# OzAmram/CaloDiffusion

Hardware: AMD Instinct MI355X
Metric: sampled showers/sec (Dataset-2, 400-step DDIM) (higher is better)
Workload: dtype f32 (convs: fp32 operands as 2-term fp16 splits on the fp16 MFMA pipe, fp32 accumulate; attention/norms fp32)

## Files before the change

calodiffusion_amd/csrc/conv_internal.h:

```cpp
#pragma once
#include "kernels_conv.h"
#include "split16.h"
#include <cstdio>
#include <cstdlib>
#include <map>
#include <string>

namespace cd {

#define MFMA32(a, b, c) __builtin_amdgcn_mfma_f32_32x32x2f32((a), (b), (c), 0, 0, 0)
#define MFMA_BF16(a, b, c) __builtin_amdgcn_mfma_f32_32x32x16_bf16(__builtin_bit_cast(bf16x8, (a)), __builtin_bit_cast(bf16x8, (b)), (c), 0, 0, 0)

typedef __bf16 bf16x8 __attribute__((ext_vector_type(8)));
typedef __bf16 bf16x2 __attribute__((ext_vector_type(2)));

__device__ __forceinline__ unsigned pack_bf16(float lo, float hi) {
  const bf16x2 v = {(__bf16)lo, (__bf16)hi};
  return __builtin_bit_cast(unsigned, v);
}
__device__ __forceinline__ void split3(const f32x4 x, u32x2& t1, u32x2& t2, u32x2& t3) {
  f32x4 r = x;
  t1 = u32x2{pack_bf16(r[0], r[1]), pack_bf16(r[2], r[3])};
  r[0] -= __uint_as_float(t1[0] << 16); r[1] -= __uint_as_float(t1[0] & 0xffff0000u);
  r[2] -= __uint_as_float(t1[1] << 16); r[3] -= __uint_as_float(t1[1] & 0xffff0000u);
// ... 21 lines not shown
struct ConvTiled3Args {
  ConvKArgs k;
  float* ch_part;
  int* status;
};
void launch_conv_tiled_f32(int VT, int CT, const ConvKArgs& a, dim3 grid, int threads, size_t lds, hipStream_t s);
void launch_conv_tiled_split16(int VT, int CT, int NTERM, const ConvTiled3Args& a, dim3 grid, int threads, size_t lds, hipStream_t s);

struct ConvFlatArgs {
  const float* in0;
  const float* in1;
  int c0, c1;
  const float* wpk;
  const float* bias;
  float* out;
  int D, H, W;
  int Do, Ho, Wo;
  int R;
  int P;
  int cout, CTtot;
  int dbg;
  const float* coef;
  int act;
  float* ch_part;
  int* status = nullptr;
  GnDefer defer;
  int coef_lds_off = 0;
  const unsigned* in_absmax = nullptr;
  const float* add_src = nullptr;
};
bool try_launch_conv3_flat(const float* in0, int c0, const float* in1, int c1, const void* wpk, const float* bias, float* out,
                           int batch, int cout, const ConvGeom& g, hipStream_t s, const ConvFusion& fu,
                           int prec );
bool launch_conv_flat_split16(int VT, int CT, int NTERM, int geo, const ConvFlatArgs& a, dim3 grid, int threads, size_t lds, hipStream_t s);

std::map<std::string, int>& tune_cache();
template <typename F>
int autotune(const std::string& key, int ncand, F&& run, hipStream_t s) {
  auto it = tune_cache().find(key);
  if (it != tune_cache().end()) return it->second;
  hipStreamCaptureStatus st = hipStreamCaptureStatusNone;
  if (getenv("CD_NO_AUTOTUNE") || hipStreamIsCapturing(s, &st) != hipSuccess || st != hipStreamCaptureStatusNone || prof::enabled())
    return -1;
  hipEvent_t e0, e1;
  CD_HIP(hipEventCreate(&e0));
  CD_HIP(hipEventCreate(&e1));
  int best = 0;
  float best_ms = 1e30f;
  for (int i = 0; i < ncand; ++i) {
    run(i);
    CD_HIP(hipEventRecord(e0, s));
    run(i);
    run(i);
    CD_HIP(hipEventRecord(e1, s));
    CD_HIP(hipEventSynchronize(e1));
    float ms = 0.f;
    CD_HIP(hipEventElapsedTime(&ms, e0, e1));
    if (getenv("CD_TUNE_VERBOSE") && atoi(getenv("CD_TUNE_VERBOSE")) > 1) std::fprintf(stderr, "[calodiff autotune]   %s cand %d: %.1f us\n", key.c_str(), i, ms * 500.f);
    if (ms < best_ms) { best_ms = ms; best = i; }
  }
  hipEventDestroy(e0);
  hipEventDestroy(e1);
  tune_cache()[key] = best;
  if (getenv("CD_TUNE_VERBOSE")) std::fprintf(stderr, "[calodiff autotune] %s -> candidate %d (%.1f us)\n", key.c_str(), best, best_ms * 500.f);
  return best;
}

// ... 2 lines not shown
```

calodiffusion_amd/csrc/kernels_conv.hip:

```cpp
#include "conv_internal.h"
#include <cstring>
#include <algorithm>
#include <vector>

namespace cd {

static int g_conv_precision = -1;
static thread_local int tl_conv_precision_override = -1;
void set_conv_precision_override(int p) { tl_conv_precision_override = p; }
int conv_precision() {
  if (tl_conv_precision_override >= 0) return tl_conv_precision_override;
  if (g_conv_precision < 0) {
    const char* e = getenv("CD_CONV_PRECISION");
    g_conv_precision = !e ? PREC_F16X2 : (!strcmp(e, "f32") ? PREC_F32 : (!strcmp(e, "bf16x3") ? PREC_BF16X3 : PREC_F16X2));
  }
  return g_conv_precision;
}
void set_conv_precision(int p) { g_conv_precision = p; }

__device__ __forceinline__ void pack_weights_elem(size_t idx, const float* __restrict__ w, float* __restrict__ wpk, int cout, int cin,
                                                  int taps, int transposed, int flip) {
  const int e = idx & 3, lane = (idx >> 2) & 63, q = (idx >> 8) & 3;
  size_t rest = idx >> 10;
  const int CT = (cout + 31) / 32;
// ... 142 lines not shown
        double per_round = (double)((resident * NW + 3) / 4) * VT;
        const double cost = rounds * per_round + 0.02 * (double)IZ * IH * g.in.w / 32.0 * rounds;
        all.push_back({cost, ConvTile{TZ, TH, NW, VT, lds}});
      }
    }
  }
  CD_REQUIRE(!all.empty(), "no convolution tiling fits in LDS (grid too wide in r?)");
  std::stable_sort(all.begin(), all.end(), [](const auto& x, const auto& y) { return x.first < y.first; });
  std::vector<ConvTile> out;
  for (auto& c : all) {
    out.push_back(c.second);
    if ((int)out.size() >= keep) break;
  }
  return out;
}

ConvKArgs conv_k_args(const ConvGeom& g, const ConvTile& t, const ConvFusion& fu, const float* in0, int c0, const float* in1, int c1,
                      const float* wpk, const float* bias, float* out, int cout) {
  ConvKArgs a;
  a.in0 = in0; a.in1 = in1; a.c0 = c0; a.c1 = c1; a.wpk = wpk; a.bias = bias; a.out = out;
  a.Din = g.in.d; a.Hin = g.in.h; a.Win = g.in.w; a.Do = g.out.d; a.Ho = g.out.h; a.Wo = g.out.w;
  a.KD = g.kd; a.KH = g.kh; a.KW = g.kw; a.SZ = g.sz; a.SH = g.sh; a.SW = g.sw;
  a.TZ = t.TZ; a.TH = t.TH; a.nTZ = (g.out.d + t.TZ - 1) / t.TZ; a.nTH = (g.out.h + t.TH - 1) / t.TH;
  a.IZ = (t.TZ - 1) * g.sz + g.kd; a.IH = (t.TH - 1) * g.sh + g.kh;
  a.cout = cout; a.CTtot = cout / 32; a.coef = fu.coef; a.act = fu.act;
  return a;
}
}

void launch_conv_mfma(const float* in0, int c0, const float* in1, int c1, const float* wpk, const float* bias, float* out,
                      int batch, int cout, const ConvGeom& g, hipStream_t s, const ConvFusion& fu_in) {
  CD_REQUIRE((!fu_in.coef && !fu_in.defer.part) || c1 == 0, "conv: a fused input normalisation needs a single (non-concatenated) source");
  if (fu_in.units) *fu_in.units = 0;
  CD_REQUIRE(c0 % 32 == 0 && c1 % 32 == 0 && c0 > 0, "conv: channel counts must be multiples of 32");
  CD_REQUIRE(cout % 32 == 0, "conv: output channels must be a multiple of 32");
  CD_REQUIRE(g.kw <= 4, "conv: r kernel extent > 4 unsupported");
  const int CTtot = cout / 32;
  const int CT = CTtot <= 3 ? CTtot : 2;
  CD_REQUIRE(CTtot % CT == 0, "conv: unsupported output channel count");
  char cat[128];
  std::snprintf(cat, sizeof cat, "conv%dx%dx%d_s%d C%d->%d @%dx%dx%d", g.kd, g.kh, g.kw, g.sh, c0 + c1, cout, g.in.d, g.in.h, g.in.w);
  const double taps = (double)g.kd * g.kh * g.kw;
  prof::Scope scope(cat, s, 2.0 * taps * (c0 + c1) * cout * (double)g.out.vox() * batch,
                    4.0 * batch * ((double)g.in.vox() * (c0 + c1) + (double)g.out.vox() * cout));
  ConvFusion fu = fu_in;
  auto materialise = [&]() {
    if (!fu.defer.part) return;
    if (fu.defer.coef_out) fu.coef_buf = fu.defer.coef_out;
    CD_REQUIRE(fu.coef_buf, "conv: deferred normalisation needs a coefficient buffer for kernels without the prologue");
    launch_gn_finalize(fu.defer.part, fu.defer.units, fu.defer.gamma, fu.defer.beta, fu.defer.add, fu.defer.add_ld, fu.coef_buf, batch,
                       fu.defer.C, fu.defer.groups, fu.defer.vox, s, fu.defer.stat_out);
    fu.coef = fu.coef_buf;
    fu.defer = GnDefer();
  };
  auto tiled = [&](int nterm, const void* w) -> bool {
    std::vector<ConvTile> cand;
    for (const ConvTile& t : conv_tile_candidates(g, batch, CT, 14, nterm == 2 ? 80 : (nterm == 3 ? 96 : 144)))
      if (nterm == 0 || (nterm == 2 ? t.VT * CT <= 2 : (t.VT <= 4 && !(CT == 3 && t.VT > 2)))) cand.push_back(t);
    if (cand.empty()) return false;
    auto launch = [&](const ConvTile& t) {
      ConvTiled3Args a3;
      a3.k = conv_k_args(g, t, fu, in0, c0, in1, c1, (const float*)w, bias, out, cout);
      const int units = a3.k.nTZ * a3.k.nTH;
      dim3 grid((unsigned)(batch * units), (unsigned)(CTtot / CT));
      if (nterm == 0) {
        launch_conv_tiled_f32(t.VT, CT, a3.k, grid, t.NW * 64, t.lds, s);
        return;
      }
      a3.status = fu.status;
      const int64_t cap = (g.out.vox() + 31) / 32;
      a3.ch_part = (fu.ch_part && units <= cap) ? fu.ch_part : nullptr;
      if (fu.units) *fu.units = a3.ch_part ? units : 0;
      const size_t red = (size_t)t.NW * CT * 32 * 2 * 4;
      launch_conv_tiled_split16(t.VT, CT, nterm, a3, grid, t.NW * 64, std::max(t.lds, red), s);
    };
    char key[192];
    if (nterm) std::snprintf(key, sizeof key, "tiled_%s %s b%d", nterm == 2 ? "f16x2" : "bf16x3", cat, batch);
    else std::snprintf(key, sizeof key, "tiled %s b%d", cat, batch);
    const int pick = autotune(key, (int)cand.size(), [&](int i) { launch(cand[i]); }, s);
    launch(cand[pick < 0 ? 0 : pick]);
    return true;
  };

  const int prec = conv_precision();
  const void* w_bf16x3 = prec != PREC_F32 ? fu.wpk_bf16x3 : nullptr;
  const void* w_f16x2 = w_bf16x3 && prec == PREC_F16X2 ? (const char*)w_bf16x3 + packed_bf16x3_bytes(c0 + c1, cout, g.kd * g.kh * g.kw) : nullptr;
  if (w_f16x2 && try_launch_conv_zslide(in0, c0, in1, c1, w_f16x2, bias, out, batch, cout, g, s, fu)) return;
  if (w_f16x2 && try_launch_conv_small(in0, c0, in1, c1, w_f16x2, bias, out, batch, cout, g, s, fu)) return;
  if (w_f16x2 && try_launch_conv3_flat(in0, c0, in1, c1, w_f16x2, bias, out, batch, cout, g, s, fu, 2)) return;
  materialise();
  if (w_bf16x3 && try_launch_conv3_flat(in0, c0, in1, c1, w_bf16x3, bias, out, batch, cout, g, s, fu, 3)) return;
  if (try_launch_conv3_flat(in0, c0, in1, c1, wpk, bias, out, batch, cout, g, s, fu, 0)) return;
  if (w_f16x2 && !fu.in_absmax && tiled(2, w_f16x2)) return;
  if (w_bf16x3 && tiled(3, w_bf16x3)) return;
  tiled(0, wpk);
}

}
```

calodiffusion_amd/csrc/kernels_conv_flat.hip:

```cpp
#include "conv_internal.h"
#include "gn_defer.h"
#include <vector>

namespace cd {

template <int VT, int CT>
__global__ void __launch_bounds__(512, (VT * CT <= 2 ? 3 : 2)) conv3_flat_kernel(ConvFlatArgs a) {
  extern __shared__ __attribute__((aligned(16))) float lds[];
  const int tid = threadIdx.x, lane = tid & 63, wave = tid >> 6, nthreads = blockDim.x;
  const int b = blockIdx.y;
  const int ct0 = blockIdx.z * CT;
  const int HW = a.H * a.W;
  const int vox = a.D * HW;
  const int v0 = blockIdx.x * a.R;
  const int vend = min(v0 + a.R, vox);
  const int zA = v0 / HW - 1;
  const int zB = (vend - 1) / HW + 1;
  const int nstage = (zB - zA + 1) * HW;
  const int NZ = a.P * HW;
  const int half = lane >> 5, col = lane & 31;
  if (tid < 16) lds[NZ * 16 + tid] = 0.f;

  int nb[VT], rowm[VT], rowp[VT], ooff[VT];
  unsigned wmask[VT];
  bool any_valid = false;
#pragma unroll
  for (int vt = 0; vt < VT; ++vt) {
    const int v = v0 + (wave * VT + vt) * 32 + col;
    const bool valid = v < vend;
    const int vv = valid ? v : v0;
    const int r = vv % HW;
    const int h = r / a.W, w = r - h * a.W;
    nb[vt] = vv - zA * HW;
    rowm[vt] = (h == 0 ? a.H - 1 : -1) * a.W;
// ... 447 lines not shown
  }
  CD_FLAT_CASE(1, 1) CD_FLAT_CASE(2, 1) CD_FLAT_CASE(3, 1) CD_FLAT_CASE(4, 1)
  CD_FLAT_CASE(1, 2) CD_FLAT_CASE(2, 2) CD_FLAT_CASE(3, 2) CD_FLAT_CASE(4, 2)
  CD_FLAT_CASE(1, 3) CD_FLAT_CASE(2, 3)
#undef CD_FLAT_CASE
  return false;
}
}

bool try_launch_conv3_flat(const float* in0, int c0, const float* in1, int c1, const void* wpk, const float* bias, float* out,
                           int batch, int cout, const ConvGeom& g, hipStream_t s, const ConvFusion& fu, int prec) {
  const bool bf16x3 = prec != 0;
  if (getenv("CD_NO_FLAT")) return false;
  int geo = -1;
  if (g.kd == 3 && g.kh == 3 && g.kw == 3 && g.sz == 1 && g.sh == 1 && g.sw == 1) geo = 0;
  else if (g.kd == 3 && g.kh == 4 && g.kw == 4 && g.sh == 2 && g.sw == 2 && (g.sz == 1 || g.sz == 2)) geo = g.sz == 2 ? 1 : 2;
  else if (g.kd == 4 && g.kh == 4 && g.kw == 4 && g.sh == 2 && g.sw == 2 && g.sz == 2) geo = 3;
  if (geo < 0 || (geo != 0 && !bf16x3)) return false;
  const Dims3 d = g.in;
  const int CTtot = cout / 32;
  const int CTmax = CTtot <= 3 ? CTtot : 2;
  if (CTtot % CTmax) return false;
  const int HW = d.h * d.w, HWo = g.out.h * g.out.w;
  const size_t vox_bytes = prec == 3 ? 96 : (prec == 2 ? 80 : 64);
  auto planes = [&](int NT) { return ((32 * NT - 1) / HWo + 1) * g.sz + g.kd; };
  auto args_for = [&](int NT) {
    ConvFlatArgs a;
    a.in0 = in0; a.in1 = in1; a.c0 = c0; a.c1 = c1; a.wpk = (const float*)wpk; a.bias = bias; a.out = out;
    a.D = d.d; a.H = d.h; a.W = d.w; a.Do = g.out.d; a.Ho = g.out.h; a.Wo = g.out.w;
    a.R = 32 * NT; a.P = planes(NT); a.cout = cout; a.CTtot = CTtot;
    a.coef = fu.coef; a.act = fu.act; a.ch_part = fu.ch_part;
    return a;
  };
  auto launch = [&](int NT, int VT, int CT) -> bool {
    if (VT < 0) {
      const int NLW = -VT;
      ConvFlatArgs a = args_for(NT);
      a.dbg = 0;
      const size_t lds = 2 * ((size_t)a.P * HW + 1) * 96 + (size_t)NT * CT * 64 * 4;
      const int ups = (int)((g.out.vox() + a.R - 1) / a.R);
      const int total = ups * batch;
      const int nblk = total < 256 ? total : 256;
      dim3 grid((unsigned)nblk, 1, (unsigned)(CTtot / CT));
      if (fu.units) *fu.units = ups;
      const int threads = (NT + NLW) * 64;
      switch (CT) {
        case 1: launch_ws_inst<1>(a, grid, threads, lds, NLW, ups, total, s, geo); break;
        case 2: launch_ws_inst<2>(a, grid, threads, lds, NLW, ups, total, s, geo); break;
        case 3: launch_ws_inst<3>(a, grid, threads, lds, NLW, ups, total, s, geo); break;
        default: return false;
      }
      return true;
    }
    ConvFlatArgs a = args_for(NT);
    a.dbg = getenv("CD_FLAT_DBG") ? atoi(getenv("CD_FLAT_DBG")) : 0;
    a.status = fu.status; a.in_absmax = fu.in_absmax;
    a.add_src = prec >= 2 && !bias ? fu.add_src : nullptr;
    size_t lds = ((size_t)a.P * HW + 1) * vox_bytes;
    const size_t red = (size_t)(NT / VT) * CT * 32 * 2 * 4;
    if (lds < red) lds = red;
    if (fu.defer.part) {
      lds = (lds + 15) & ~(size_t)15;
      a.defer = fu.defer;
      a.coef_lds_off = (int)lds;
      lds += (size_t)fu.defer.C * 16 + gn_defer_scratch_bytes(fu.defer.C);
      if (lds > 160 * 1024) return false;
    }
    dim3 grid((unsigned)((g.out.vox() + a.R - 1) / a.R), (unsigned)batch, (unsigned)(CTtot / CT));
    if (fu.units) *fu.units = (int)grid.x;
    const int threads = (NT / VT) * 64;
    const bool launched = prec != 0 ? launch_conv_flat_split16(VT, CT, prec, geo, a, grid, threads, lds, s)
                                    : launch_conv_flat_f32(VT, CT, a, grid, threads, lds, s);
    if (!launched) return false;
    if (a.add_src && fu.add_done) *fu.add_done = 1;
    return true;
  };
  if (const char* ov = getenv("CD_FLAT_TILE")) {
    int nt, vt;
    if (sscanf(ov, "%d,%d", &nt, &vt) == 2 && nt % vt == 0 && nt / vt <= 8 && vt * CTmax <= 8 &&
        ((size_t)planes(nt) * HW + 1) * vox_bytes <= 160 * 1024 && (prec != 2 || vt * CTmax <= 4))
      return launch(nt, vt, CTmax);
  }
  static const int kCand[][2] = {{8, 2}, {4, 1}, {8, 1}, {12, 3}, {16, 2}, {16, 4}, {4, 2}, {6, 2}, {6, 3}, {2, 1},
                                 {3, 1}, {1, 1}, {2, 2}, {12, 2}, {8, 4}, {6, 1}, {3, 3}};
  struct Cand { int nt, vt, ct; };
  std::vector<Cand> cand;
  const bool small = g.out.vox() * batch <= 64 * 1024;
  for (int pass = 0; pass < (small && CTmax > 1 ? 2 : 1); ++pass) {
    const int CT = pass == 0 ? CTmax : 1;
    for (auto& c : kCand) {
      const int NT = c[0], VT = c[1];
      if (VT * CT > 8 || (CT == 3 && VT > 2)) continue;
      if (prec == 2 && VT * CT > 4) continue;
      static const bool no_extra_waves = getenv("CD_FLAT_NO_EXTRA_WAVES") != nullptr;
      const bool extra_ok = !no_extra_waves && g.out.vox() <= 128 && VT == 1 && NT <= 8;
      if ((int64_t)32 * (NT - 1) >= g.out.vox() && !extra_ok) continue;
      if (((size_t)planes(NT) * HW + 1) * vox_bytes > 150 * 1024) continue;
      if (pass == 1 && NT > 4) continue;
      cand.push_back({NT, VT, CT});
    }
  }
  if (prec == 3 && !getenv("CD_NO_WS")) {
    static const int kWs[][2] = {{8, 4}, {8, 2}, {4, 2}, {4, 4}, {8, 3}, {6, 2}, {2, 2}, {3, 1}, {1, 1}, {2, 1}};
    for (auto& c : kWs) {
      const int NMW = c[0], NLW = c[1];
      if ((int64_t)32 * (NMW - 1) >= g.out.vox()) continue;
      const size_t lds = 2 * ((size_t)planes(NMW) * HW + 1) * 96 + (size_t)NMW * CTmax * 64 * 4;
      if (lds > 160 * 1024 - 256) continue;
      cand.push_back({NMW, -NLW, CTmax});
    }
  }
  if (cand.empty()) return false;
  char key[192];
  std::snprintf(key, sizeof key, "flat%s g%d %dx%dx%d c%d+%d->%d b%d", prec == 3 ? "_bf16x3" : (prec == 2 ? "_f16x2" : "_f32"), geo,
                d.d, d.h, d.w, c0, c1, cout, batch);
  const int pick = autotune(key, (int)cand.size(), [&](int i) { launch(cand[i].nt, cand[i].vt, cand[i].ct); }, s);
  const Cand& c = cand[pick < 0 ? 0 : pick];
  return launch(c.nt, c.vt, c.ct);
}

}
```

calodiffusion_amd/csrc/kernels_conv_flat16.hip:

```cpp
#include "conv_internal.h"
#include "gn_defer.h"

namespace cd {

template <int VT, int CT, int KD, int KH, int KW, int SZ, int SXY, int NTERM>
__global__ void __launch_bounds__(512, (VT * CT * (NTERM == 2 ? 2 : 1) <= 2 ? 3 : 2)) conv3_flat_bf16x3_kernel(ConvFlatArgs a) {
  extern __shared__ __attribute__((aligned(16))) float lds[];
  char* ldsb = (char*)lds;
  constexpr int T = KD * KH * KW;
  constexpr int VB = NTERM == 3 ? 96 : 80;
  constexpr int WS = 64 * NTERM;
  const int tid = threadIdx.x, lane = tid & 63, wave = tid >> 6, nthreads = blockDim.x;
  const int b = blockIdx.y;
  const int ct0 = blockIdx.z * CT;
  const int HW = a.H * a.W;
  const int vox = a.D * HW;
  const int HWo = a.Ho * a.Wo;
  const int voxo = a.Do * HWo;
  const int v0 = blockIdx.x * a.R;
  const int vend = min(v0 + a.R, voxo);
  const float inv_hwo = 1.f / (float)HWo, inv_wo = 1.f / (float)a.Wo;
  auto fdiv = [](int x, float inv) { return (int)(((float)x + 0.5f) * inv); };
  const int zA = fdiv(v0, inv_hwo) * SZ - 1;
  const int zB = fdiv(vend - 1, inv_hwo) * SZ + KD - 2;
  const int nstage = (zB - zA + 1) * HW;
  const int NZ = a.P * HW;
  const int half = lane >> 5, col = lane & 31;
  if (a.defer.part) gn_defer_to_lds(a.defer, b, (float*)(ldsb + a.coef_lds_off), ldsb + a.coef_lds_off + a.defer.C * 16);
  const bool normed = a.coef || a.defer.part;
  if (tid < VB / 4) ((float*)(ldsb + (size_t)NZ * VB))[tid] = 0.f;

  int nb[VT], rowoff[VT][KH], ooff[VT];
  unsigned wmask[VT];
  bool any_valid = false;
#pragma unroll
  for (int vt = 0; vt < VT; ++vt) {
    const int v = v0 + (wave * VT + vt) * 32 + col;
    const bool valid = v < vend;
    const int vv = valid ? v : v0;
    const int oz = fdiv(vv, inv_hwo);
    const int r = vv - oz * HWo;
    const int oh = fdiv(r, inv_wo), ow = r - oh * a.Wo;
    const int ih0 = oh * SXY, iw0 = ow * SXY;
    nb[vt] = (oz * SZ - 1 - zA) * HW + ih0 * a.W + iw0;
    unsigned m = 0;
#pragma unroll
    for (int kh = 0; kh < KH; ++kh) {
      int ih = ih0 + kh - 1;
      ih = ih < 0 ? ih + a.H : (ih >= a.H ? ih - a.H : ih);
      ih = ih >= a.H ? ih - a.H : ih;
      rowoff[vt][kh] = (ih - ih0) * a.W;
    }
#pragma unroll
    for (int kw = 0; kw < KW; ++kw) {
      const int iw = iw0 + kw - 1;
      if (valid && iw >= 0 && iw < a.W) m |= 1u << kw;
    }
    wmask[vt] = m;
    ooff[vt] = valid ? v * a.cout : -1;
    any_valid |= valid;
  }
  const bool wave_active = __any(any_valid);

  f32x16 acc[VT][CT], accB[NTERM == 2 ? VT : 1][NTERM == 2 ? CT : 1];
#pragma unroll
  for (int vt = 0; vt < VT; ++vt)
#pragma unroll
    for (int ct = 0; ct < CT; ++ct)
#pragma unroll
      for (int r = 0; r < 16; ++r) {
// ... 6 lines not shown
  if (NTERM == 2 && a.in_absmax) pow2_scale_for(*a.in_absmax, &gscale, &ginv);
  const int nsub = (a.c0 + a.c1) >> 4;
  const int gbase = zA * HW;
  const int nslots = nstage * 4;

  auto tap_voxel = [&](int vt, int tap) -> int {
#ifdef CD_FLAT_ABL_TAPS
    return nb[vt] + tap;
#endif
    const int kz = tap / (KH * KW), kh = (tap / KW) % KH, kw = tap % KW;
    const int n = nb[vt] + kz * HW + rowoff[vt][kh] + kw - 1;
    return ((wmask[vt] >> kw) & 1u) ? n : NZ;
  };

  for (int sc = 0; sc < nsub; ++sc) {
    const float* src;
    int ldc, coff;
    if (sc * 16 < a.c0) {
      src = a.in0; ldc = a.c0; coff = sc * 16;
    } else {
      src = a.in1; ldc = a.c1; coff = sc * 16 - a.c0;
    }
    const int pq = tid & 3;
    src += (size_t)b * vox * ldc + coff + pq * 4;
    f32x4 cf[4];
    if (a.defer.part) {
#pragma unroll
      for (int e = 0; e < 4; ++e) cf[e] = *(const f32x4*)(ldsb + a.coef_lds_off + (sc * 16 + pq * 4 + e) * 16);
    } else if (a.coef) {
#pragma unroll
      for (int e = 0; e < 4; ++e) cf[e] = *(const f32x4*)(a.coef + ((size_t)b * (a.c0 + a.c1) + sc * 16 + pq * 4 + e) * 4);
    }
    __syncthreads();
    for (int s0 = tid; s0 < ((a.dbg & 1) ? 0 : nslots); s0 += 4 * nthreads) {
      f32x4 val[4];
#pragma unroll
      for (int k = 0; k < 4; ++k) {
        const int sidx = s0 + k * nthreads;
        const int g = gbase + (sidx >> 2);
        val[k] = f32x4{0.f, 0.f, 0.f, 0.f};
        if (sidx < nslots && g >= 0 && g < vox) {
          val[k] = *(const f32x4*)(src + (size_t)g * ldc);
          if (normed) {
#pragma unroll
            for (int e = 0; e < 4; ++e) {
              float t = cf[e][0] * val[k][e] + cf[e][1];
              if (a.act) t = cd_fast_silu(t);
              val[k][e] = t + cf[e][2];
            }
          }
        }
      }
#pragma unroll
      for (int k = 0; k < 4; ++k) {
        const int sidx = s0 + k * nthreads;
        if (sidx < nslots) {
          char* d = ldsb + (size_t)(sidx >> 2) * VB + pq * 8;
          if (NTERM == 3) {
            u32x2 t1, t2, t3;
            split3(val[k], t1, t2, t3);
            *(u32x2*)d = t1;
            *(u32x2*)(d + 32) = t2;
            *(u32x2*)(d + 64) = t3;
          } else {
            const f32x4 vs = val[k] * gscale;
            amax = fmaxf(amax, fmaxf(fmaxf(fabsf(vs[0]), fabsf(vs[1])), fmaxf(fabsf(vs[2]), fabsf(vs[3]))));
            u32x2 t1, t2;
            split2(vs, t1, t2);
            *(u32x2*)d = t1;
            *(u32x2*)(d + 32) = t2;
          }
        }
      }
    }
    __syncthreads();
    if (!wave_active || (a.dbg & 2)) continue;

#pragma unroll
    for (int vt = 0; vt < VT; ++vt) asm volatile("" : "+v"(nb[vt]));

    const u32x4* wq = (const u32x4*)a.wpk + ((size_t)sc * T * a.CTtot + ct0) * WS + lane;
#ifndef CD_FLAT_WD
#define CD_FLAT_WD 3
#endif
#ifndef CD_FLAT_AD
#define CD_FLAT_AD 2
#endif
    constexpr bool DEEP = NTERM == 2;
    constexpr int WD = DEEP ? CD_FLAT_WD : 1, AD = DEEP ? CD_FLAT_AD : 1;
    u32x4 bw[WD + 1][CT][NTERM], av[AD + 1][VT][NTERM];
    auto load_w = [&](int tap) {
#pragma unroll
      for (int ct = 0; ct < CT; ++ct)
#pragma unroll
        for (int t = 0; t < NTERM; ++t) bw[tap % (WD + 1)][ct][t] = wq[((size_t)tap * a.CTtot + ct) * WS + t * 64];
    };
    auto load_a = [&](int tap) {
#pragma unroll
      for (int vt = 0; vt < VT; ++vt) {
        const char* p = ldsb + (size_t)tap_voxel(vt, tap) * VB + half * 16;
#pragma unroll
        for (int t = 0; t < NTERM; ++t) av[tap % (AD + 1)][vt][t] = *(const u32x4*)(p + t * 32);
      }
    };
#pragma unroll
    for (int t0 = 0; t0 < WD; ++t0) load_w(t0);
#pragma unroll
    for (int t0 = 0; t0 < AD; ++t0) load_a(t0);
#pragma unroll
    for (int tap = 0; tap < T; ++tap) {
      if (tap + WD < T) load_w(tap + WD);
      if (tap + AD < T) load_a(tap + AD);
      __builtin_amdgcn_sched_barrier(0);
      const int wc = tap % (WD + 1), ac = tap % (AD + 1);
#pragma unroll
      for (int vt = 0; vt < VT; ++vt)
#pragma unroll
        for (int ct = 0; ct < CT; ++ct) {
          if (NTERM == 3) {
            f32x16 c = acc[vt][ct];
            c = MFMA_BF16(av[ac][vt][NTERM - 1], bw[wc][ct][0], c);
            c = MFMA_BF16(av[ac][vt][1], bw[wc][ct][1], c);
            c = MFMA_BF16(av[ac][vt][0], bw[wc][ct][NTERM - 1], c);
            c = MFMA_BF16(av[ac][vt][1], bw[wc][ct][0], c);
            c = MFMA_BF16(av[ac][vt][0], bw[wc][ct][1], c);
            c = MFMA_BF16(av[ac][vt][0], bw[wc][ct][0], c);
            acc[vt][ct] = c;
          } else {
            acc[vt][ct] = MFMA_F16(av[ac][vt][0], bw[wc][ct][0], acc[vt][ct]);
            accB[vt][ct] = MFMA_F16(av[ac][vt][0], bw[wc][ct][1], accB[vt][ct]);
            accB[vt][ct] = MFMA_F16(av[ac][vt][1], bw[wc][ct][0], accB[vt][ct]);
          }
        }
    }
  }

  if (NTERM == 2) {
#pragma unroll
    for (int vt = 0; vt < VT; ++vt)
#pragma unroll
      for (int ct = 0; ct < CT; ++ct)
#pragma unroll
        for (int r = 0; r < 16; ++r) acc[vt][ct][r] = (acc[vt][ct][r] + accB[vt][ct][r] * (1.f / 2048.f)) * ginv;
  }
  if (NTERM == 2 && a.status && amax > 65504.f) atomicOr(a.status, 1);
  float* outb = a.out + (size_t)b * voxo * a.cout;
  float bv[CT];
#pragma unroll
  for (int ct = 0; ct < CT; ++ct) bv[ct] = a.bias ? a.bias[(ct0 + ct) * 32 + col] : 0.f;
  if (a.add_src) {
    const float* addb = a.add_src + (size_t)b * voxo * a.cout;
#pragma unroll
    for (int vt = 0; vt < VT; ++vt) {
      float ad[16][CT];
#pragma unroll
      for (int r = 0; r < 16; ++r) {
        const int off = __shfl(ooff[vt], (r & 3) + 8 * (r >> 2) + 4 * half, 64);
#pragma unroll
        for (int ct = 0; ct < CT; ++ct) ad[r][ct] = off >= 0 ? addb[off + (ct0 + ct) * 32 + col] : 0.f;
      }
#pragma unroll
      for (int r = 0; r < 16; ++r)
#pragma unroll
        for (int ct = 0; ct < CT; ++ct) acc[vt][ct][r] += ad[r][ct];
    }
  }
#pragma unroll
  for (int vt = 0; vt < VT; ++vt) {
#pragma unroll
    for (int r = 0; r < 16; ++r) {
      const int row = (r & 3) + 8 * (r >> 2) + 4 * half;
      const int off = __shfl(ooff[vt], row, 64);
      if (off >= 0) {
#pragma unroll
        for (int ct = 0; ct < CT; ++ct) outb[off + (ct0 + ct) * 32 + col] = acc[vt][ct][r] + bv[ct];
      }
    }
  }
// ... 9 lines not shown
        const bool ok = __shfl(ooff[vt], row, 64) >= 0;
#pragma unroll
        for (int ct = 0; ct < CT; ++ct) {
          const float v = ok ? acc[vt][ct][r] + bv[ct] : 0.f;
          s1[ct] += v;
          s2[ct] += v * v;
        }
      }
    __syncthreads();
    const int nw = nthreads >> 6;
#pragma unroll
    for (int ct = 0; ct < CT; ++ct) {
      const float t1 = s1[ct] + __shfl_xor(s1[ct], 32, 64), t2 = s2[ct] + __shfl_xor(s2[ct], 32, 64);
      if (half == 0) {
        lds[((wave * CT + ct) * 32 + col) * 2] = t1;
        lds[((wave * CT + ct) * 32 + col) * 2 + 1] = t2;
      }
    }
    __syncthreads();
    for (int i = tid; i < CT * 32; i += nthreads) {
      float t1 = 0.f, t2 = 0.f;
      for (int w = 0; w < nw; ++w) {
        t1 += lds[((w * CT * 32) + i) * 2];
        t2 += lds[((w * CT * 32) + i) * 2 + 1];
      }
      float* dst = a.ch_part + (((size_t)b * gridDim.x + blockIdx.x) * a.cout + ct0 * 32 + i) * 2;
      dst[0] = t1;
      dst[1] = t2;
    }
  }
}

namespace {
template <int VT, int CT, int KD, int KH, int KW, int SZ, int SXY, int NTERM>
void launch_flat3_geo(const ConvFlatArgs& a, dim3 grid, int threads, size_t lds, hipStream_t s) {
  static bool attr_set = false;
  if (!attr_set) {
    CD_HIP(hipFuncSetAttribute((const void*)conv3_flat_bf16x3_kernel<VT, CT, KD, KH, KW, SZ, SXY, NTERM>,
                               hipFuncAttributeMaxDynamicSharedMemorySize, 160 * 1024));
    attr_set = true;
  }
  hipLaunchKernelGGL((conv3_flat_bf16x3_kernel<VT, CT, KD, KH, KW, SZ, SXY, NTERM>), grid, dim3(threads), lds, s, a);
  CD_HIP(hipGetLastError());
}
template <int VT, int CT, int NTERM>
void launch_flat3_inst(const ConvFlatArgs& a, dim3 grid, int threads, size_t lds, hipStream_t s, int geo = 0) {
  if (geo == 0) launch_flat3_geo<VT, CT, 3, 3, 3, 1, 1, NTERM>(a, grid, threads, lds, s);
  else if (geo == 1) launch_flat3_geo<VT, CT, 3, 4, 4, 2, 2, NTERM>(a, grid, threads, lds, s);
  else if (geo == 2) launch_flat3_geo<VT, CT, 3, 4, 4, 1, 2, NTERM>(a, grid, threads, lds, s);
  else launch_flat3_geo<VT, CT, 4, 4, 4, 2, 2, NTERM>(a, grid, threads, lds, s);
}
}

bool launch_conv_flat_split16(int VT, int CT, int NTERM, int geo, const ConvFlatArgs& a, dim3 grid, int threads, size_t lds, hipStream_t s) {
#define CD_FLAT_CASE(V, C)                                                                 \
  if (VT == V && CT == C) {                                                                \
    if (NTERM == 3) launch_flat3_inst<V, C, 3>(a, grid, threads, lds, s, geo);             \
    else if constexpr (V * C <= 4) launch_flat3_inst<V, C, 2>(a, grid, threads, lds, s, geo); \
    else return false;                                                                     \
    return true;                                                                           \
  }
  CD_FLAT_CASE(1, 1) CD_FLAT_CASE(2, 1) CD_FLAT_CASE(3, 1) CD_FLAT_CASE(4, 1)
  CD_FLAT_CASE(1, 2) CD_FLAT_CASE(2, 2) CD_FLAT_CASE(3, 2) CD_FLAT_CASE(4, 2)
  CD_FLAT_CASE(1, 3) CD_FLAT_CASE(2, 3)
#undef CD_FLAT_CASE
  return false;
}

}
```

calodiffusion_amd/csrc/ops.hip:

```cpp
#include "plan_internal.h"

namespace cd {

__global__ void to_cl_kernel(const float* __restrict__ src, float* __restrict__ dst, int channels, int64_t vox) {
  const int b = blockIdx.y;
  const int64_t total = vox * channels;
  for (int64_t i = (int64_t)blockIdx.x * 256 + threadIdx.x; i < total; i += (int64_t)gridDim.x * 256) {
    const int c = (int)(i % channels);
    const int64_t v = i / channels;
    dst[(size_t)b * total + i] = src[(size_t)b * total + (size_t)c * vox + v];
  }
}
__global__ void to_planar_kernel(const float* __restrict__ src, float* __restrict__ dst, int channels, int64_t vox) {
  const int b = blockIdx.y;
  const int64_t total = vox * channels;
  for (int64_t i = (int64_t)blockIdx.x * 256 + threadIdx.x; i < total; i += (int64_t)gridDim.x * 256) {
    const int64_t v = i % vox;
    const int c = (int)(i / vox);
    dst[(size_t)b * total + i] = src[(size_t)b * total + (size_t)v * channels + c];
  }
}
static void launch_transpose_to_cl(const float* ncdhw, float* ndhwc, int batch, int channels, int64_t vox, hipStream_t s) {
  int64_t bx = (vox * channels + 255) / 256;
  if (bx > 1024) bx = 1024;
// ... 6 lines not shown
  hipLaunchKernelGGL(to_planar_kernel, dim3((unsigned)bx, batch), dim3(256), 0, s, ndhwc, ncdhw, channels, vox);
  CD_HIP(hipGetLastError());
}

}

extern "C" {

static AbsmaxWords op_absmax_words(Arena& ws, hipStream_t s) {
  constexpr size_t kWords = 8;
  unsigned* w = ws.get<unsigned>(kWords);
  CD_HIP(hipMemsetAsync(w, 0, sizeof(unsigned) * kWords, s));
  return AbsmaxWords{w, w + kWords};
}
size_t cd_op_scratch_bytes(int batch, int max_channels, int64_t max_voxels) {
  return (size_t)256 * 256 * 64 * 4 * 4 + (size_t)batch * 64 * 64 * 16 + (size_t)batch * max_channels * max_voxels * 4 + (1 << 20);
}

int cd_op_to_channels_last(const float* ncdhw, float* ndhwc, int batch, int channels, int64_t voxels, void* stream) {
  return guarded([&] { launch_transpose_to_cl(ncdhw, ndhwc, batch, channels, voxels, (hipStream_t)stream); });
}
int cd_op_to_ncdhw(const float* ndhwc, float* ncdhw, int batch, int channels, int64_t voxels, void* stream) {
  return guarded([&] { launch_transpose_to_planar(ndhwc, ncdhw, batch, channels, voxels, (hipStream_t)stream); });
}

int cd_op_cyl_conv(const float* x0, int c0, const float* x1, int c1, const float* w, const float* bias, float* y,
                   int batch, int cout, const int32_t dims_in[3], const int32_t kernel[3], const int32_t stride[3],
                   void* scratch, void* stream) {
  return guarded([&] {
    CD_REQUIRE(x0 && w && y && scratch, "null argument");
    hipStream_t s = (hipStream_t)stream;
    const int taps = kernel[0] * kernel[1] * kernel[2];
    float* wpk = (float*)scratch;
    launch_pack_weights(w, wpk, cout, c0 + c1, taps, false, s);
    const Dims3 din{dims_in[0], dims_in[1], dims_in[2]};
    if (taps == 1) {
      PointwiseArgs a;
      a.in0 = x0; a.ld0 = c0; a.c0 = c0; a.in1 = x1; a.ld1 = c1; a.c1 = c1; a.wpk = wpk; a.bias = bias; a.out = y;
      a.batch = batch; a.cout = cout; a.vox = din.vox();
      launch_pointwise(a, s);
    } else {
      CD_REQUIRE(cout % 32 == 0, "cout must be a multiple of 32");
      ConvGeom g;
      g.in = din;
      g.kd = kernel[0]; g.kh = kernel[1]; g.kw = kernel[2]; g.sz = stride[0]; g.sh = stride[1]; g.sw = stride[2];
      g.out = Dims3{(din.d + 2 - g.kd) / g.sz + 1, (din.h + 2 - g.kh) / g.sh + 1, (din.w + 2 - g.kw) / g.sw + 1};
      ConvFusion fu;
      if (taps == 27 || taps == 48) {
        float* w3 = wpk + packed_weight_floats(c0 + c1, cout, taps);
        launch_pack_weights_split16(w, w3, cout, c0 + c1, taps, s);
        fu.wpk_bf16x3 = w3;
      }
      launch_conv_mfma(x0, c0, x1, c1, wpk, bias, y, batch, cout, g, s, fu);
    }
  });
}

int cd_op_zslide_conv(const float* x, int cin, const float* w, const float* bias, float* y, float* ch_part, int* units, int batch,
                      int cout, const int32_t dims[3], int chunks, void* scratch, void* stream) {
  return guarded([&] {
    CD_REQUIRE(x && w && y && ch_part && units && scratch && chunks >= 0, "bad argument");
    CD_REQUIRE(cin % 32 == 0 && cout % 32 == 0, "channel counts must be multiples of 32");
    hipStream_t s = (hipStream_t)stream;
    launch_pack_weights_f16x2(w, scratch, cout, cin, 27, s);
    const Dims3 d{dims[0], dims[1], dims[2]};
    ConvGeom g{d, d, 3, 3, 3, 1, 1, 1};
    ConvFusion fu;
    int u = 0;
    fu.act = 1; fu.ch_part = ch_part; fu.units = &u; fu.zs_chunks = chunks;
    CD_REQUIRE(try_launch_conv_zslide(x, cin, nullptr, 0, scratch, bias, y, batch, cout, g, s, fu) && u > 0,
               "this grid is not eligible for the z-slide kernel");
    *units = u;
  });
}

int cd_op_cyl_conv_transpose(const float* x, const float* w, const float* bias, float* y, int batch, int channels,
                             const int32_t dims_in[3], int kernel_z, int stride_z, const int32_t out_pad[3],
                             void* scratch, void* stream) {
  return guarded([&] {
    CD_REQUIRE(x && w && y && scratch, "null argument");
    CD_REQUIRE(out_pad[0] == 0, "z output padding is always 0 (models.py:339)");
    hipStream_t s = (hipStream_t)stream;
// ... 153 lines not shown
```

Measured before the change: 92.57.

## Add tap-split (split-K over taps) variants of flat f16x2 conv kernel

Adds a KS template parameter to the flat split16 conv kernel so several wave groups each handle a disjoint slice of the kernel taps for the same output tile. Their partial accumulators are reduced through LDS before the epilogue. The variants are offered as extra autotune candidates for the 3x4x4 geometries, to raise parallelism on small-voxel layers. The change also relaxes the channel requirement to multiples of 16 for 4x4 kernels on the f16x2 path. The cost is more LDS use, an extra reduction and barrier step, and a longer autotune search.

```diff
diff --git a/calodiffusion_amd/csrc/conv_internal.h b/calodiffusion_amd/csrc/conv_internal.h
--- a/calodiffusion_amd/csrc/conv_internal.h
+++ b/calodiffusion_amd/csrc/conv_internal.h
@@ -77,7 +77,9 @@
 bool try_launch_conv3_flat(const float* in0, int c0, const float* in1, int c1, const void* wpk, const float* bias, float* out,
                            int batch, int cout, const ConvGeom& g, hipStream_t s, const ConvFusion& fu,
                            int prec );
-bool launch_conv_flat_split16(int VT, int CT, int NTERM, int geo, const ConvFlatArgs& a, dim3 grid, int threads, size_t lds, hipStream_t s);
+bool launch_conv_flat_split16(int VT, int CT, int NTERM, int geo, const ConvFlatArgs& a, dim3 grid, int threads, size_t lds, hipStream_t s,
+                              int KS = 1);
+bool conv_flat_tapsplit_offered(int VT, int CT, int NTERM, int geo, int KS);
 
 std::map<std::string, int>& tune_cache();
 template <typename F>
diff --git a/calodiffusion_amd/csrc/kernels_conv.hip b/calodiffusion_amd/csrc/kernels_conv.hip
--- a/calodiffusion_amd/csrc/kernels_conv.hip
+++ b/calodiffusion_amd/csrc/kernels_conv.hip
@@ -198,7 +198,9 @@
                       int batch, int cout, const ConvGeom& g, hipStream_t s, const ConvFusion& fu_in) {
   CD_REQUIRE((!fu_in.coef && !fu_in.defer.part) || c1 == 0, "conv: a fused input normalisation needs a single (non-concatenated) source");
   if (fu_in.units) *fu_in.units = 0;
-  CD_REQUIRE(c0 % 32 == 0 && c1 % 32 == 0 && c0 > 0, "conv: channel counts must be multiples of 32");
+  const bool half_chunk = c0 % 32 != 0 || c1 % 32 != 0;
+  CD_REQUIRE(c0 % 16 == 0 && c1 % 16 == 0 && c0 > 0 && (!half_chunk || (g.kh == 4 && g.kw == 4)),
+             "conv: channel counts must be multiples of 32");
   CD_REQUIRE(cout % 32 == 0, "conv: output channels must be a multiple of 32");
   CD_REQUIRE(g.kw <= 4, "conv: r kernel extent > 4 unsupported");
   const int CTtot = cout / 32;
@@ -254,6 +256,7 @@
   if (w_f16x2 && try_launch_conv_zslide(in0, c0, in1, c1, w_f16x2, bias, out, batch, cout, g, s, fu)) return;
   if (w_f16x2 && try_launch_conv_small(in0, c0, in1, c1, w_f16x2, bias, out, batch, cout, g, s, fu)) return;
   if (w_f16x2 && try_launch_conv3_flat(in0, c0, in1, c1, w_f16x2, bias, out, batch, cout, g, s, fu, 2)) return;
+  CD_REQUIRE(!half_chunk, "conv: channel counts must be multiples of 32 (16-channel multiples run on the f16x2 flat kernel only)");
   materialise();
   if (w_bf16x3 && try_launch_conv3_flat(in0, c0, in1, c1, w_bf16x3, bias, out, batch, cout, g, s, fu, 3)) return;
   if (try_launch_conv3_flat(in0, c0, in1, c1, wpk, bias, out, batch, cout, g, s, fu, 0)) return;
diff --git a/calodiffusion_amd/csrc/kernels_conv_flat.hip b/calodiffusion_amd/csrc/kernels_conv_flat.hip
--- a/calodiffusion_amd/csrc/kernels_conv_flat.hip
+++ b/calodiffusion_amd/csrc/kernels_conv_flat.hip
@@ -1,5 +1,6 @@
 #include "conv_internal.h"
 #include "gn_defer.h"
+#include <algorithm>
 #include <vector>
 
 namespace cd {
@@ -513,7 +514,7 @@
     a.coef = fu.coef; a.act = fu.act; a.ch_part = fu.ch_part;
     return a;
   };
-  auto launch = [&](int NT, int VT, int CT) -> bool {
+  auto launch = [&](int NT, int VT, int CT, int KS = 1) -> bool {
     if (VT < 0) {
       const int NLW = -VT;
       ConvFlatArgs a = args_for(NT);
@@ -538,8 +539,10 @@
     a.status = fu.status; a.in_absmax = fu.in_absmax;
     a.add_src = prec >= 2 && !bias ? fu.add_src : nullptr;
     size_t lds = ((size_t)a.P * HW + 1) * vox_bytes;
-    const size_t red = (size_t)(NT / VT) * CT * 32 * 2 * 4;
+    size_t red = (size_t)KS * (NT / VT) * CT * 32 * 2 * 4;
+    if (KS > 1) red = std::max(red, (size_t)(KS - 1) * NT * CT * 4096);
     if (lds < red) lds = red;
+    if (lds > 160 * 1024) return false;
     if (fu.defer.part) {
       lds = (lds + 15) & ~(size_t)15;
       a.defer = fu.defer;
@@ -549,22 +552,24 @@
     }
     dim3 grid((unsigned)((g.out.vox() + a.R - 1) / a.R), (unsigned)batch, (unsigned)(CTtot / CT));
     if (fu.units) *fu.units = (int)grid.x;
-    const int threads = (NT / VT) * 64;
-    const bool launched = prec != 0 ? launch_conv_flat_split16(VT, CT, prec, geo, a, grid, threads, lds, s)
+    const int threads = KS * (NT / VT) * 64;
+    const bool launched = prec != 0 ? launch_conv_flat_split16(VT, CT, prec, geo, a, grid, threads, lds, s, KS)
                                     : launch_conv_flat_f32(VT, CT, a, grid, threads, lds, s);
     if (!launched) return false;
     if (a.add_src && fu.add_done) *fu.add_done = 1;
     return true;
   };
   if (const char* ov = getenv("CD_FLAT_TILE")) {
-    int nt, vt;
-    if (sscanf(ov, "%d,%d", &nt, &vt) == 2 && nt % vt == 0 && nt / vt <= 8 && vt * CTmax <= 8 &&
+    int nt, vt, ks = 1;
+    const int nf = sscanf(ov, "%d,%d,%d", &nt, &vt, &ks);
+    if (nf < 3 || ks == 1 || !conv_flat_tapsplit_offered(vt, 1, prec, geo, ks) || ks * nt / vt > 8) ks = 1;
+    if (nf >= 2 && nt > 0 && vt > 0 && nt % vt == 0 && nt / vt <= 8 && vt * CTmax <= 8 &&
         ((size_t)planes(nt) * HW + 1) * vox_bytes <= 160 * 1024 && (prec != 2 || vt * CTmax <= 4))
-      return launch(nt, vt, CTmax);
+      return launch(nt, vt, ks > 1 ? 1 : CTmax, ks);
   }
   static const int kCand[][2] = {{8, 2}, {4, 1}, {8, 1}, {12, 3}, {16, 2}, {16, 4}, {4, 2}, {6, 2}, {6, 3}, {2, 1},
                                  {3, 1}, {1, 1}, {2, 2}, {12, 2}, {8, 4}, {6, 1}, {3, 3}};
-  struct Cand { int nt, vt, ct; };
+  struct Cand { int nt, vt, ct, ks; };
   std::vector<Cand> cand;
   const bool small = g.out.vox() * batch <= 64 * 1024;
   for (int pass = 0; pass < (small && CTmax > 1 ? 2 : 1); ++pass) {
@@ -578,7 +583,20 @@
       if ((int64_t)32 * (NT - 1) >= g.out.vox() && !extra_ok) continue;
       if (((size_t)planes(NT) * HW + 1) * vox_bytes > 150 * 1024) continue;
       if (pass == 1 && NT > 4) continue;
-      cand.push_back({NT, VT, CT});
+      cand.push_back({NT, VT, CT, 1});
+    }
+  }
+  static const int kSplit[][2] = {{4, 2}, {3, 2}, {2, 4}, {2, 2}, {1, 4}};
+  bool has_split = false;
+  for (int pass = 0; pass < (small && CTmax > 1 ? 2 : 1); ++pass) {
+    const int CT = pass == 0 ? CTmax : 1;
+    for (auto& c : kSplit) {
+      const int NT = c[0], KS = c[1];
+      if (!conv_flat_tapsplit_offered(1, CT, prec, geo, KS)) continue;
+      if ((int64_t)32 * (NT - 1) >= g.out.vox()) continue;
+      if (((size_t)planes(NT) * HW + 1) * vox_bytes > 150 * 1024) continue;
+      cand.push_back({NT, 1, CT, KS});
+      has_split = true;
     }
   }
   if (prec == 3 && !getenv("CD_NO_WS")) {
@@ -588,16 +606,21 @@
       if ((int64_t)32 * (NMW - 1) >= g.out.vox()) continue;
       const size_t lds = 2 * ((size_t)planes(NMW) * HW + 1) * 96 + (size_t)NMW * CTmax * 64 * 4;
       if (lds > 160 * 1024 - 256) continue;
-      cand.push_back({NMW, -NLW, CTmax});
+      cand.push_back({NMW, -NLW, CTmax, 1});
     }
   }
   if (cand.empty()) return false;
   char key[192];
-  std::snprintf(key, sizeof key, "flat%s g%d %dx%dx%d c%d+%d->%d b%d", prec == 3 ? "_bf16x3" : (prec == 2 ? "_f16x2" : "_f32"), geo,
-                d.d, d.h, d.w, c0, c1, cout, batch);
-  const int pick = autotune(key, (int)cand.size(), [&](int i) { launch(cand[i].nt, cand[i].vt, cand[i].ct); }, s);
+  std::snprintf(key, sizeof key, "flat%s%s g%d %dx%dx%d c%d+%d->%d b%d", prec == 3 ? "_bf16x3" : (prec == 2 ? "_f16x2" : "_f32"),
+                has_split ? "+ks" : "", geo, d.d, d.h, d.w, c0, c1, cout, batch);
+  const int pick = autotune(key, (int)cand.size(), [&](int i) { launch(cand[i].nt, cand[i].vt, cand[i].ct, cand[i].ks); }, s);
   const Cand& c = cand[pick < 0 ? 0 : pick];
-  return launch(c.nt, c.vt, c.ct);
-}
-
-}
+  if (getenv("CD_TUNE_VERBOSE") && pick >= 0) {
+    static std::map<std::string, int> said;
+    if (said.emplace(key, pick).second)
+      std::fprintf(stderr, "[calodiff autotune]   %s = nt %d vt %d ct %d ks %d\n", key, c.nt, c.vt, c.ct, c.ks);
+  }
+  return launch(c.nt, c.vt, c.ct, c.ks);
+}
+
+}
diff --git a/calodiffusion_amd/csrc/kernels_conv_flat16.hip b/calodiffusion_amd/csrc/kernels_conv_flat16.hip
--- a/calodiffusion_amd/csrc/kernels_conv_flat16.hip
+++ b/calodiffusion_amd/csrc/kernels_conv_flat16.hip
@@ -1,16 +1,25 @@
 #include "conv_internal.h"
 #include "gn_defer.h"
+#include <type_traits>
 
 namespace cd {
 
-template <int VT, int CT, int KD, int KH, int KW, int SZ, int SXY, int NTERM>
-__global__ void __launch_bounds__(512, (VT * CT * (NTERM == 2 ? 2 : 1) <= 2 ? 3 : 2)) conv3_flat_bf16x3_kernel(ConvFlatArgs a) {
+template <int VT, int CT, int KD, int KH, int KW, int SZ, int SXY, int NTERM, int KS = 1>
+__global__ void __launch_bounds__(512, (KS > 1 ? 2 : (VT * CT * (NTERM == 2 ? 2 : 1) <= 2 ? 3 : 2)))
+conv3_flat_bf16x3_kernel(ConvFlatArgs a) {
+  static_assert(KS == 1 || (NTERM == 2 && VT == 1 && CT == 1 && (KS == 2 || KS == 4) && (KD * KH * KW) % KS == 0), "tap-split instances");
   extern __shared__ __attribute__((aligned(16))) float lds[];
   char* ldsb = (char*)lds;
   constexpr int T = KD * KH * KW;
   constexpr int VB = NTERM == 3 ? 96 : 80;
   constexpr int WS = 64 * NTERM;
   const int tid = threadIdx.x, lane = tid & 63, wave = tid >> 6, nthreads = blockDim.x;
+  int wt = wave, kr = 0;
+  if constexpr (KS > 1) {
+    const int w = __builtin_amdgcn_readfirstlane(wave), nwt = a.R >> 5;
+    kr = (w >= nwt ? 1 : 0) + (w >= 2 * nwt ? 1 : 0) + (w >= 3 * nwt ? 1 : 0);
+    wt = w - kr * nwt;
+  }
   const int b = blockIdx.y;
   const int ct0 = blockIdx.z * CT;
   const int HW = a.H * a.W;
@@ -35,7 +44,7 @@
   bool any_valid = false;
 #pragma unroll
   for (int vt = 0; vt < VT; ++vt) {
-    const int v = v0 + (wave * VT + vt) * 32 + col;
+    const int v = v0 + (wt * VT + vt) * 32 + col;
     const bool valid = v < vend;
     const int vv = valid ? v : v0;
     const int oz = fdiv(vv, inv_hwo);
@@ -108,10 +117,11 @@
       for (int e = 0; e < 4; ++e) cf[e] = *(const f32x4*)(a.coef + ((size_t)b * (a.c0 + a.c1) + sc * 16 + pq * 4 + e) * 4);
     }
     __syncthreads();
-    for (int s0 = tid; s0 < ((a.dbg & 1) ? 0 : nslots); s0 += 4 * nthreads) {
-      f32x4 val[4];
-#pragma unroll
-      for (int k = 0; k < 4; ++k) {
+    constexpr int LB = KS > 1 ? 8 : 4;
+    for (int s0 = tid; s0 < ((a.dbg & 1) ? 0 : nslots); s0 += LB * nthreads) {
+      f32x4 val[LB];
+#pragma unroll
+      for (int k = 0; k < LB; ++k) {
         const int sidx = s0 + k * nthreads;
         const int g = gbase + (sidx >> 2);
         val[k] = f32x4{0.f, 0.f, 0.f, 0.f};
@@ -128,7 +138,7 @@
         }
       }
 #pragma unroll
-      for (int k = 0; k < 4; ++k) {
+      for (int k = 0; k < LB; ++k) {
         const int sidx = s0 + k * nthreads;
         if (sidx < nslots) {
           char* d = ldsb + (size_t)(sidx >> 2) * VB + pq * 8;
@@ -179,35 +189,64 @@
         for (int t = 0; t < NTERM; ++t) av[tap % (AD + 1)][vt][t] = *(const u32x4*)(p + t * 32);
       }
     };
-#pragma unroll
-    for (int t0 = 0; t0 < WD; ++t0) load_w(t0);
-#pragma unroll
-    for (int t0 = 0; t0 < AD; ++t0) load_a(t0);
-#pragma unroll
-    for (int tap = 0; tap < T; ++tap) {
-      if (tap + WD < T) load_w(tap + WD);
-      if (tap + AD < T) load_a(tap + AD);
-      __builtin_amdgcn_sched_barrier(0);
-      const int wc = tap % (WD + 1), ac = tap % (AD + 1);
-#pragma unroll
-      for (int vt = 0; vt < VT; ++vt)
-#pragma unroll
-        for (int ct = 0; ct < CT; ++ct) {
-          if (NTERM == 3) {
-            f32x16 c = acc[vt][ct];
-            c = MFMA_BF16(av[ac][vt][NTERM - 1], bw[wc][ct][0], c);
-            c = MFMA_BF16(av[ac][vt][1], bw[wc][ct][1], c);
-            c = MFMA_BF16(av[ac][vt][0], bw[wc][ct][NTERM - 1], c);
-            c = MFMA_BF16(av[ac][vt][1], bw[wc][ct][0], c);
-            c = MFMA_BF16(av[ac][vt][0], bw[wc][ct][1], c);
-            c = MFMA_BF16(av[ac][vt][0], bw[wc][ct][0], c);
-            acc[vt][ct] = c;
-          } else {
-            acc[vt][ct] = MFMA_F16(av[ac][vt][0], bw[wc][ct][0], acc[vt][ct]);
-            accB[vt][ct] = MFMA_F16(av[ac][vt][0], bw[wc][ct][1], accB[vt][ct]);
-            accB[vt][ct] = MFMA_F16(av[ac][vt][1], bw[wc][ct][0], accB[vt][ct]);
+    if constexpr (KS == 1) {
+#pragma unroll
+      for (int t0 = 0; t0 < WD; ++t0) load_w(t0);
+#pragma unroll
+      for (int t0 = 0; t0 < AD; ++t0) load_a(t0);
+#pragma unroll
+      for (int tap = 0; tap < T; ++tap) {
+        if (tap + WD < T) load_w(tap + WD);
+        if (tap + AD < T) load_a(tap + AD);
+        __builtin_amdgcn_sched_barrier(0);
+        const int wc = tap % (WD + 1), ac = tap % (AD + 1);
+#pragma unroll
+        for (int vt = 0; vt < VT; ++vt)
+#pragma unroll
+          for (int ct = 0; ct < CT; ++ct) {
+            if (NTERM == 3) {
+              f32x16 c = acc[vt][ct];
+              c = MFMA_BF16(av[ac][vt][NTERM - 1], bw[wc][ct][0], c);
+              c = MFMA_BF16(av[ac][vt][1], bw[wc][ct][1], c);
+              c = MFMA_BF16(av[ac][vt][0], bw[wc][ct][NTERM - 1], c);
+              c = MFMA_BF16(av[ac][vt][1], bw[wc][ct][0], c);
+              c = MFMA_BF16(av[ac][vt][0], bw[wc][ct][1], c);
+              c = MFMA_BF16(av[ac][vt][0], bw[wc][ct][0], c);
+              acc[vt][ct] = c;
+            } else {
+              acc[vt][ct] = MFMA_F16(av[ac][vt][0], bw[wc][ct][0], acc[vt][ct]);
+              accB[vt][ct] = MFMA_F16(av[ac][vt][0], bw[wc][ct][1], accB[vt][ct]);
+              accB[vt][ct] = MFMA_F16(av[ac][vt][1], bw[wc][ct][0], accB[vt][ct]);
+            }
+          }
+      }
+    } else {
+      auto run_taps = [&](auto range) {
+        constexpr int T0 = decltype(range)::value * (T / KS), T1 = T0 + T / KS;
+#pragma unroll
+        for (int t0 = 0; t0 < WD; ++t0) load_w(T0 + t0);
+#pragma unroll
+        for (int t0 = 0; t0 < AD; ++t0) load_a(T0 + t0);
+#pragma unroll
+        for (int tap = T0; tap < T1; ++tap) {
+          if (tap + WD < T1) load_w(tap + WD);
+          if (tap + AD < T1) load_a(tap + AD);
+          __builtin_amdgcn_sched_barrier(0);
+          const int wc = tap % (WD + 1), ac = tap % (AD + 1);
+#pragma unroll
+          for (int ct = 0; ct < CT; ++ct) {
+            acc[0][ct] = MFMA_F16(av[ac][0][0], bw[wc][ct][0], acc[0][ct]);
+            accB[0][ct] = MFMA_F16(av[ac][0][0], bw[wc][ct][1], accB[0][ct]);
+            accB[0][ct] = MFMA_F16(av[ac][0][1], bw[wc][ct][0], accB[0][ct]);
           }
         }
+      };
+      if (kr == 0) run_taps(std::integral_constant<int, 0>{});
+      else if (kr == 1) run_taps(std::integral_constant<int, 1>{});
+      if constexpr (KS == 4) {
+        if (kr == 2) run_taps(std::integral_constant<int, 2>{});
+        else if (kr == 3) run_taps(std::integral_constant<int, 3>{});
+      }
     }
   }
 
@@ -220,6 +259,34 @@
         for (int r = 0; r < 16; ++r) acc[vt][ct][r] = (acc[vt][ct][r] + accB[vt][ct][r] * (1.f / 2048.f)) * ginv;
   }
   if (NTERM == 2 && a.status && amax > 65504.f) atomicOr(a.status, 1);
+  if constexpr (KS > 1) {
+    const int nwt = a.R >> 5;
+    __syncthreads();
+    if (kr > 0) {
+      f32x4* red = (f32x4*)ldsb + (size_t)((kr - 1) * nwt + wt) * CT * 256 + lane;
+#pragma unroll
+      for (int ct = 0; ct < CT; ++ct)
+#pragma unroll
+        for (int q = 0; q < 4; ++q)
+          red[(ct * 4 + q) * 64] = f32x4{acc[0][ct][4 * q], acc[0][ct][4 * q + 1], acc[0][ct][4 * q + 2], acc[0][ct][4 * q + 3]};
+      ooff[0] = -1;
+    }
+    __syncthreads();
+    if (kr == 0) {
+#pragma unroll
+      for (int k = 1; k < KS; ++k) {
+        const f32x4* red = (const f32x4*)ldsb + (size_t)((k - 1) * nwt + wt) * CT * 256 + lane;
+#pragma unroll
+        for (int ct = 0; ct < CT; ++ct)
+#pragma unroll
+          for (int q = 0; q < 4; ++q) {
+            const f32x4 t = red[(ct * 4 + q) * 64];
+#pragma unroll
+            for (int e = 0; e < 4; ++e) acc[0][ct][4 * q + e] += t[e];
+          }
+      }
+    }
+  }
   float* outb = a.out + (size_t)b * voxo * a.cout;
   float bv[CT];
 #pragma unroll
@@ -295,15 +362,15 @@
 }
 
 namespace {
-template <int VT, int CT, int KD, int KH, int KW, int SZ, int SXY, int NTERM>
+template <int VT, int CT, int KD, int KH, int KW, int SZ, int SXY, int NTERM, int KS = 1>
 void launch_flat3_geo(const ConvFlatArgs& a, dim3 grid, int threads, size_t lds, hipStream_t s) {
   static bool attr_set = false;
   if (!attr_set) {
-    CD_HIP(hipFuncSetAttribute((const void*)conv3_flat_bf16x3_kernel<VT, CT, KD, KH, KW, SZ, SXY, NTERM>,
+    CD_HIP(hipFuncSetAttribute((const void*)conv3_flat_bf16x3_kernel<VT, CT, KD, KH, KW, SZ, SXY, NTERM, KS>,
                                hipFuncAttributeMaxDynamicSharedMemorySize, 160 * 1024));
     attr_set = true;
   }
-  hipLaunchKernelGGL((conv3_flat_bf16x3_kernel<VT, CT, KD, KH, KW, SZ, SXY, NTERM>), grid, dim3(threads), lds, s, a);
+  hipLaunchKernelGGL((conv3_flat_bf16x3_kernel<VT, CT, KD, KH, KW, SZ, SXY, NTERM, KS>), grid, dim3(threads), lds, s, a);
   CD_HIP(hipGetLastError());
 }
 template <int VT, int CT, int NTERM>
@@ -313,9 +380,25 @@
   else if (geo == 2) launch_flat3_geo<VT, CT, 3, 4, 4, 1, 2, NTERM>(a, grid, threads, lds, s);
   else launch_flat3_geo<VT, CT, 4, 4, 4, 2, 2, NTERM>(a, grid, threads, lds, s);
 }
-}
-
-bool launch_conv_flat_split16(int VT, int CT, int NTERM, int geo, const ConvFlatArgs& a, dim3 grid, int threads, size_t lds, hipStream_t s) {
+template <int KS>
+void launch_flat3_tapsplit(const ConvFlatArgs& a, dim3 grid, int threads, size_t lds, hipStream_t s, int geo) {
+  if (geo == 1) launch_flat3_geo<1, 1, 3, 4, 4, 2, 2, 2, KS>(a, grid, threads, lds, s);
+  else launch_flat3_geo<1, 1, 3, 4, 4, 1, 2, 2, KS>(a, grid, threads, lds, s);
+}
+}
+
+bool conv_flat_tapsplit_offered(int VT, int CT, int NTERM, int geo, int KS) {
+  return NTERM == 2 && (geo == 1 || geo == 2) && VT == 1 && CT == 1 && (KS == 2 || KS == 4);
+}
+
+bool launch_conv_flat_split16(int VT, int CT, int NTERM, int geo, const ConvFlatArgs& a, dim3 grid, int threads, size_t lds, hipStream_t s,
+                              int KS) {
+  if (KS != 1) {
+    if (!conv_flat_tapsplit_offered(VT, CT, NTERM, geo, KS)) return false;
+    if (KS == 2) launch_flat3_tapsplit<2>(a, grid, threads, lds, s, geo);
+    else launch_flat3_tapsplit<4>(a, grid, threads, lds, s, geo);
+    return true;
+  }
 #define CD_FLAT_CASE(V, C)                                                                 \
   if (VT == V && CT == C) {                                                                \
     if (NTERM == 3) launch_flat3_inst<V, C, 3>(a, grid, threads, lds, s, geo);             \
diff --git a/calodiffusion_amd/csrc/ops.hip b/calodiffusion_amd/csrc/ops.hip
--- a/calodiffusion_amd/csrc/ops.hip
+++ b/calodiffusion_amd/csrc/ops.hip
@@ -62,7 +62,8 @@
     hipStream_t s = (hipStream_t)stream;
     const int taps = kernel[0] * kernel[1] * kernel[2];
     float* wpk = (float*)scratch;
-    launch_pack_weights(w, wpk, cout, c0 + c1, taps, false, s);
+    const bool half_chunk = (c0 % 32 || c1 % 32) && c0 % 16 == 0 && c1 % 16 == 0 && taps == 48;
+    if (!half_chunk) launch_pack_weights(w, wpk, cout, c0 + c1, taps, false, s);
     const Dims3 din{dims_in[0], dims_in[1], dims_in[2]};
     if (taps == 1) {
       PointwiseArgs a;
@@ -77,7 +78,7 @@
       g.out = Dims3{(din.d + 2 - g.kd) / g.sz + 1, (din.h + 2 - g.kh) / g.sh + 1, (din.w + 2 - g.kw) / g.sw + 1};
       ConvFusion fu;
       if (taps == 27 || taps == 48) {
-        float* w3 = wpk + packed_weight_floats(c0 + c1, cout, taps);
+        float* w3 = wpk + packed_weight_floats((c0 + c1 + 31) & ~31, cout, taps);
         launch_pack_weights_split16(w, w3, cout, c0 + c1, taps, s);
         fu.wpk_bf16x3 = w3;
       }
```

Result: no change. 93.49, median of 6 (+1.0%).
